# rahulrangers/P2P-Gossip-Simulation-NS3

Measured on AMD Instinct MI355X. Metric: share-deliveries/sec (edge events) at 10M nodes, 1/2/4/8 GPUs; % HBM/MFMA peak, higher is better.
Workload: dtype u64

## Files before the change

include/gossip.h:

```cpp
#ifndef GOSSIP_H
#define GOSSIP_H

#include <stdint.h>

#ifdef __cplusplus
extern "C" {
#endif

#define GOSSIP_OK 0
#define GOSSIP_EINVAL (-1)
#define GOSSIP_EHIP (-2)
#define GOSSIP_ENOMEM (-3)
#define GOSSIP_ESTATE (-4)
#define GOSSIP_ECAPACITY (-5)

const char* gossip_last_error(void);
const char* gossip_version(void);

int64_t gossip_seconds_to_ns(double seconds);
int64_t gossip_milliseconds_to_ns(double ms);

typedef struct gossip_topology gossip_topology;

#define GOSSIP_TOPO_EXACT 0
// ... 151 lines not shown
    uint64_t pull_sat_skips;
    uint32_t pull_sat;
    uint32_t pad0;
    uint64_t window_early_retires;
    uint64_t young_list_lines;
    uint64_t pull_items;
    uint64_t pull_gather_items;
    uint64_t dense_fused_launches;
    uint32_t young_grid;
    uint32_t young_skip_ticks;
    uint64_t pull_push_tiles;
    uint64_t pull_pushw_tiles;
    uint64_t pull_marks;
    uint64_t young_idle_ticks;
    uint64_t pull_fold_rows;
} gossip_counters;
int gossip_engine_get_counters(gossip_engine* e, gossip_counters* c);
int gossip_engine_get_rehearsal(gossip_engine* e, uint32_t ranges, double* pull_ms, double* pack_ms,
                                double* unpack_ms, uint64_t* msg_bytes, uint64_t* ticks);
int gossip_engine_get_rehearsal_peak(gossip_engine* e, uint32_t ranges, uint64_t* msg_bytes_max);
int gossip_engine_reset_timing(gossip_engine* e);

uint64_t gossip_engine_trace_size(const gossip_engine* e);
int gossip_engine_get_trace(const gossip_engine* e, uint32_t* node, uint32_t* share_id,
                            int64_t* tick, uint32_t* hop, uint8_t* via_recv);

void gossip_engine_destroy(gossip_engine* e);

int64_t gossip_format_event_log(const gossip_topology* t, uint64_t num_events,
                                const gossip_gen_event* ev, uint64_t num_trace,
// ... 25 lines not shown
```

p2p-gossip-simulation-ns3_amd/csrc/engine.hip:

```cpp
#include <hip/hip_runtime.h>
#include <hipcub/hipcub.hpp>
#include <rccl/rccl.h>

#include <algorithm>
#include <atomic>
#include <cstdlib>
#include <cstring>
#include <memory>
#include <mutex>
#include <new>
#include <numeric>
#include <queue>
#include <string>
#include <chrono>
#include <thread>
#include <type_traits>
#include <unordered_map>
#include <vector>

#include "internal.h"

using gossip::set_error;

namespace {
// ... 58 lines not shown
    const unsigned long long* nz_cur;
    unsigned long long* nz_next;
    uint32_t ntw;
    uint32_t v0 = 0;
    uint32_t shared_out = 0;
    uint32_t keep_lds = 0;
    uint32_t gate_seen = 1;
    const uint16_t* ptile = nullptr;
    uint32_t nptile = 0;
    unsigned long long* sat = nullptr;
    const unsigned long long* tmask = nullptr;
    const unsigned long long* mark_cur = nullptr;
    unsigned long long* mark_next = nullptr;
    uint32_t short_batch = 0;
    uint32_t fold = 0;
};

__device__ __forceinline__ uint64_t group_of(uint32_t b, uint64_t gm, uint64_t gs) {
    const uint64_t below = gs & (b == 63u ? ~0ull : ((2ull << b) - 1ull));
    const uint32_t s = 63u - (uint32_t)__builtin_clzll(below);
    const uint64_t above = gs & (s == 63u ? 0ull : ~((2ull << s) - 1ull));
    const uint64_t upto = above ? ((above & (~above + 1ull)) - 1ull) : ~0ull;
    return gm & upto & ~((1ull << s) - 1ull);
}
__device__ __forceinline__ uint64_t group_fix(uint64_t nw, uint64_t seen, uint64_t gm,
                                              uint64_t gs) {
    uint64_t todo = nw & gm;
    while (todo) {
        const uint64_t grp = group_of((uint32_t)__builtin_ctzll(todo), gm, gs);
        if (seen & grp) {
// ... 28 lines not shown
    return (uint32_t)__builtin_amdgcn_readlane((int)v, (int)src);
}
__device__ __forceinline__ uint32_t wave_sum32(uint32_t x) {
    x += (uint32_t)__builtin_amdgcn_update_dpp(0, (int)x, 0xB1, 0xF, 0xF, false);
    x += (uint32_t)__builtin_amdgcn_update_dpp(0, (int)x, 0x4E, 0xF, 0xF, false);
    x += (uint32_t)__builtin_amdgcn_update_dpp(0, (int)x, 0x141, 0xF, 0xF, false);
    x += (uint32_t)__builtin_amdgcn_update_dpp(0, (int)x, 0x140, 0xF, 0xF, false);
    return lane_read(x, 0) + lane_read(x, 16) + lane_read(x, 32) + lane_read(x, 48);
}

#include "pull_kernel.h"
#include "dense_kernel.h"
#include "young_kernel.h"

constexpr uint64_t kPullNtBytes = 16ull << 30;

int64_t env_option(const char* name, int64_t dflt) {
    const char* e = std::getenv(name);
    return e && *e ? (int64_t)std::atoll(e) : dflt;
}

uint64_t pull_grid_cap(bool nt, int64_t ov) {
    if (ov > 0) return (uint64_t)ov;
    return nt ? 16384ull : 4096ull;
}

constexpr int kWideLanes = 32;

bool pull_sp(int lpw, int epn, const PullArgs& a);
template <int LPW, bool SHORT, bool FOLD>
void launch_pull_sp(bool nt, bool push, uint32_t grid, size_t lds, hipStream_t s, const PullArgs& a) {
    if (nt && push)
        k_pull<LPW, 1, true, true, true, SHORT, FOLD><<<grid, 256, lds, s>>>(a);
    else if (nt)
        k_pull<LPW, 1, true, true, false, SHORT, FOLD><<<grid, 256, lds, s>>>(a);
    else if (push)
        k_pull<LPW, 1, false, true, true, SHORT, FOLD><<<grid, 256, lds, s>>>(a);
    else
        k_pull<LPW, 1, false, true, false, SHORT, FOLD><<<grid, 256, lds, s>>>(a);
}
template <int LPW, int EPN>
void launch_pull_t(bool nt, uint32_t grid, size_t lds, hipStream_t s, const PullArgs& a) {
    if constexpr (LPW == 32 && EPN == 1) {
        if (pull_sp(LPW, EPN, a)) {
            const bool push = a.mark_cur != nullptr || a.mark_next != nullptr;
            if (a.short_batch && a.fold)
                launch_pull_sp<LPW, true, true>(nt, push, grid, lds, s, a);
            else if (a.short_batch)
                launch_pull_sp<LPW, true, false>(nt, push, grid, lds, s, a);
            else if (a.fold)
                launch_pull_sp<LPW, false, true>(nt, push, grid, lds, s, a);
            else
                launch_pull_sp<LPW, false, false>(nt, push, grid, lds, s, a);
            return;
        }
    }
    if constexpr ((LPW == 64 || LPW == 32 || LPW == 16) && EPN == 1) {
        if (nt) {
            k_pull<LPW, 1, true><<<grid, 256, lds, s>>>(a);
            return;
// ... 481 lines not shown
    int64_t opt_seen_fold = -1;
    std::vector<int64_t> tile_lastborn;
    std::vector<int64_t> tile_foldw;
    std::vector<uint8_t> tile_folded;
    bool fold_barred = false;
    std::vector<uint8_t> fold_launch;
    std::vector<uint8_t> tr_foldw, tr_seenf;
    bool any_folded() const {
        for (size_t tl = 0; tl < tile_folded.size() && tl < tile_alloc.size(); tl++)
            if (tile_alloc[tl] && tile_folded[tl]) return true;
        return false;
    }
    int64_t opt_pull_push = -1;
    int64_t opt_peer_order = 1;
    int64_t opt_pull_batch = 0;
    std::vector<int64_t> tile_pushw;
    std::vector<std::vector<std::pair<int64_t, uint32_t>>> tile_births;
    void note_birth(uint32_t tl, int64_t t) {
        auto& h = tile_births[tl];
        if (!h.empty() && h.back().first == t)
            h.back().second++;
        else
            h.emplace_back(t, 1u);
    }
    unsigned long long* d_mark[2] = {nullptr, nullptr};
    uint64_t push_tiles = 0, pushw_tiles = 0;
    int64_t mark_tick = INT64_MIN;
    uint64_t mark_launches = 0;
    bool push_write(uint32_t tl, int64_t t) const;
    double frontier_entries(uint32_t tl, int64_t t) const;
    std::vector<int64_t> tile_inj_prev;
    std::vector<uint32_t> tile_cols;
    std::vector<double> hop_front;
    uint32_t last_lpw = 0, last_dense_tiles = 0;
    uint64_t sat_launches = 0;
    bool dense_row_hop(uint32_t tl, int64_t hop) const;
    void mark_inject(uint32_t tl, int64_t t) {
        if (tile_last_inject[tl] != t) {
            tile_inj_prev[tl] = tile_last_inject[tl];
            tile_last_inject[tl] = t;
        }
    }
    int64_t opt_young_nt = 1;
    int64_t opt_young_skip = -1;
    bool skip_wr_last = false;
    uint64_t skip_ticks = 0;
    int64_t opt_young_idle = 1;
    uint64_t idle_ticks = 0;
// ... 106 lines not shown
    int decode_trace(int64_t t);
    hipEvent_t get_event();
};

gossip_engine::~gossip_engine() {
    if (xstream) hipStreamSynchronize(xstream);
    if (stream) hipStreamSynchronize(stream);
    for (auto& p : timers) {
        hipEventDestroy(p.first);
        hipEventDestroy(p.second);
    }
    for (auto e : event_pool) hipEventDestroy(e);
    hipFree(d_rowptr); hipFree(d_col); hipFree(d_deg);
    hipFree(d_rowptr_c); hipFree(d_col_c); hipFree(d_degc);
    for (int k = 0; k < 4; k++) { hipFree(d_smask[k]); hipHostFree(h_smask[k]); }
    hipFree(d_F[0]); hipFree(d_F[1]); hipFree(d_seen_mem); hipFree(d_nz[0]); hipFree(d_nz[1]); hipFree(d_sat); hipFree(d_mark[0]); hipFree(d_mark[1]); hipFree(d_Ab); hipFree(d_FT[0]); hipFree(d_FT[1]); hipFree(d_snz[0]); hipFree(d_snz[1]); hipFree(d_snz[2]); hipFree(d_tix); hipFree(d_inc); hipFree(d_ftmsg); hipFree(d_ftrecv);
    hipFree(d_recv); hipFree(d_gen); hipFree(d_effgen); hipFree(d_sent); hipFree(d_phase_ts);
    hipFree(d_live[0]); hipFree(d_live[1]); hipFree(d_live[2]); hipFree(d_scalars); hipFree(d_acct);
    hipFree(d_msg); hipFree(d_cnt); hipFree(d_scan_tmp); hipFree(d_recv_msgs); hipFree(d_sizes);
    hipFree(d_tot); hipFree(d_ovf); hipHostFree(h_tot);
    for (int k = 0; k < kRing; k++) { hipFree(d_ptile[k]); hipHostFree(h_ptile[k]); }
    for (int k = 0; k < kRing; k++) { hipFree(d_tmask[k]); hipHostFree(h_tmask[k]); }
    hipFree(d_slot[0]); hipFree(d_slot[1]);
    hipFree(d_rev); hipFree(d_hint[0]); hipFree(d_hint[1]); hipFree(d_ylist); hipFree(d_ywork);
    for (int k = 0; k < kRing; k++) { hipFree(d_young[k]); hipHostFree(h_young[k]); }
    for (auto& p : timers_young) {
        hipEventDestroy(p.first);
        hipEventDestroy(p.second);
    }
    if (comm && !aborted.load()) ncclCommDestroy(comm);
    for (int k = 0; k < kRing; k++) {
// ... 320 lines not shown
    d_seen = d_seen_mem - (uint64_t)seen_lo * stride;
    HIP_TRY(hipMemsetAsync(d_F[0], 0, bm, stream));
    HIP_TRY(hipMemsetAsync(d_F[1], 0, bm, stream));
    HIP_TRY(hipMemsetAsync(d_seen_mem, 0, bm_seen, stream));
    {
        ntw = (stride + 1023u) / 1024u;
        const size_t nzb = (size_t)n * ntw * 8;
        for (int k = 0; k < 2; k++) {
            HIP_TRY(hipMalloc(&d_nz[k], nzb));
            HIP_TRY(hipMemsetAsync(d_nz[k], 0, nzb, stream));
        }
        if (!dense) {
            HIP_TRY(hipMalloc(&d_sat, nzb));
            HIP_TRY(hipMemsetAsync(d_sat, 0, nzb, stream));
        }
        if (!dense && row_count == 1 && !handshake)
            for (int k = 0; k < 2; k++) {
                HIP_TRY(hipMalloc(&d_mark[k], ((size_t)n + 64) / 64 * 8));
                HIP_TRY(hipMemsetAsync(d_mark[k], 0, ((size_t)n + 64) / 64 * 8, stream));
            }
    }
    {
        hop_front.clear();
        const double avg_deg = n ? (double)nnz / n : 0.0;
        double reached = n ? 1.0 / n : 0.0, front = reached;
        for (int h = 0; h < 64 && front > 0.0; h++) {
            hop_front.push_back(front);
            const double nx = (1.0 - reached) * (1.0 - std::exp(-avg_deg * front));
            reached += nx;
            front = nx;
        }
    }
    HIP_TRY(hipMalloc(&d_recv, (size_t)n * 4));
    HIP_TRY(hipMalloc(&d_gen, (size_t)n * 4));
    HIP_TRY(hipMalloc(&d_effgen, (size_t)n * 4));
    HIP_TRY(hipMalloc(&d_sent, (size_t)n * 8));
    {
        const unsigned long long init[6] = {~0ull, 0ull, 0ull, 0ull, ~0ull, 0ull};
        HIP_TRY(hipMalloc(&d_phase_ts, sizeof(init)));
        HIP_TRY(hipMemcpy(d_phase_ts, init, sizeof(init), hipMemcpyHostToDevice));
    }
    HIP_TRY(hipMemsetAsync(d_recv, 0, (size_t)n * 4, stream));
// ... 311 lines not shown
    return (double)tile_cols[tl] * hop_front[(size_t)hop] >= kDenseRowBits;
}

double gossip_engine::frontier_entries(uint32_t tl, int64_t t) const {
    double e = 0.0;
    for (const auto& b : tile_births[tl]) {
        const int64_t h = t - b.first;
        if (h >= 0 && h < (int64_t)hop_front.size()) e += (double)b.second * hop_front[(size_t)h];
    }
    return e;
}
bool gossip_engine::push_write(uint32_t tl, int64_t t) const {
    if (opt_pull_push == 1) return true;
    const double avg_deg = n ? (double)nnz / n : 0.0;
    return 1.0 - std::exp(-frontier_entries(tl, t) * avg_deg) < kPushFrac;
}

uint32_t gossip_engine::soft_cap() const {
    const uint32_t margin = std::max<uint32_t>(2u * kTileWords, stride / 16u / kTileWords * kTileWords);
    return stride > margin ? stride - margin : 0u;
}

int gossip_engine::retire_early(int64_t t) {
    if (row_count > 1 || batch) return GOSSIP_OK;
    const int64_t kt = t - 1;
    const int ls = (int)(((kt % kRing) + kRing) % kRing);
    if (kt < tick0 || !live_pending[ls] || live_tick[ls] != kt) return GOSSIP_OK;
    HIP_TRY(hipEventSynchronize(live_done[ls]));
    live_pending[ls] = false;
    early_retires++;
// ... 335 lines not shown
    const bool fold_ok = opt_seen_fold != 0 && sat_on && dr_used && !fold_barred && !handshake && !batch &&
                         !link_timing && opt_rehearse_rows <= 1;
    auto sat_window = [&](uint32_t wb) {
        const uint32_t wl = std::min(kPullLdsWords, hw - wb);
        int lpw = 8;
        while (lpw < 64 && 2 * lpw < (int)wl) lpw *= 2;
        if (lpw == 64) return true;
        const double avg_deg = n ? (double)nnz / n : 0.0;
        return !(lpw * 2 <= 64 && 8 < avg_deg);
    };
    if (trace) {
        tr_foldw.assign(hw / kTileWords, 0);
        tr_seenf.assign(hw / kTileWords, 0);
    }
    fold_launch.assign((hw + kPullLdsWords - 1) / kPullLdsWords, 0);
    if (sat_used || dr_used) {
        if (TM_WORDS * ntw > tmask_cap) {
            HIP_TRY(hipStreamSynchronize(stream));
            const uint32_t cap = TM_WORDS * std::max<uint32_t>(ntw, 8u);
            for (int k = 0; k < kRing; k++) {
                hipFree(d_tmask[k]);
                hipHostFree(h_tmask[k]);
                HIP_TRY(hipMalloc(&d_tmask[k], (size_t)cap * 8));
                HIP_TRY(hipHostMalloc(&h_tmask[k], (size_t)cap * 8, hipHostMallocDefault));
            }
            tmask_cap = cap;
        }
        unsigned long long* TM = h_tmask[slot];
        std::memset(TM, 0, (size_t)TM_WORDS * ntw * 8);
        const uint32_t ntiles = hw / kTileWords;
// ... 29 lines not shown
                m[TM_FOLDW] |= bit;
                tile_foldw[tl] = t;
                tile_folded[tl] = 1;
            }
            if (seenf || foldw) {
                fold_launch[tl * kTileWords / kPullLdsWords] = 1;
                if (trace) {
                    tr_foldw[tl] = foldw;
                    tr_seenf[tl] = seenf;
                }
            }
            if (opt_pull_batch && !fresh && tile_cols[tl] &&
                frontier_entries(tl, t - 1) >= 0.5 * (double)tile_cols[tl]) {
                m[TM_SHORT] |= bit;
                short_any = true;
            }
            if (push_on && !dr && !fresh && tile_pushw[tl] == t - 1) {
                m[TM_PUSH] |= bit;
                push_tiles++;
            }
            if (light_next && !dw && push_write(tl, t)) {
                m[TM_PUSHW] |= bit;
                pushw_any = true;
            }
            tile_listed[tl] = t;
        }
        if (dr_used && young)
            for (uint32_t i = 0; i < ny_leave; i++) {
                YoungTile& y = YP->yt[YP->lv[i]];
                if (dense_row_hop(y.tile, t - tile_first[y.tile])) {
// ... 103 lines not shown
                    c.ptile = d_ptile[slot] + pt_off[li];
                    c.nptile = pt_cnt[li];
                }
                int lpw = 8;
                while (lpw < 64 && 2 * lpw < (int)c.wact) lpw *= 2;
                const bool wide_window = lpw == 64 && split_edges;
                if (wide_window) lpw = kWideLanes;
                int epn = 1;
                while (split_edges && !wide_window && lpw * epn * 2 <= 64 && epn * 8 < avg_deg) epn *= 2;
                size_t extra_lds = 0;
                if (c.ptile && epn == 1 && (sat_used || dr_used)) {
                    c.tmask = d_tmask[slot];
                    c.sat = sat_used ? d_sat : nullptr;
                    c.short_batch = short_any ? 1u : 0u;
                    c.fold = (sat_used && li < fold_launch.size() && fold_launch[li]) ? 1u : 0u;
                    if (push_on && pull_sp(lpw, epn, c)) {
                        c.mark_cur = mark_tick == t - 1 ? d_mark[(t - 1) & 1] : nullptr;
                        mark_launches += c.mark_cur != nullptr;
                        c.mark_next = pushw_any ? d_mark[t & 1] : nullptr;
                        if (c.mark_next)
                            for (uint32_t tl = wb / kTileWords; tl < (wb + c.wact) / kTileWords; tl++)
                                if ((h_tmask[slot][(size_t)TM_WORDS * (tl >> 6) + TM_PUSHW] >> (tl & 63u)) & 1ull) {
                                    tile_pushw[tl] = t;
                                    pushw_tiles++;
                                }
                    }
                    extra_lds = kPullSatLds + ((c.mark_cur || c.mark_next) ? kPullPushLds : 0);
                    sat_launches += sat_used;
                    if (sat_used)
                        for (uint32_t tl = wb / kTileWords; tl < (wb + c.wact) / kTileWords; tl++)
// ... 923 lines not shown
        e->opt_pull_gate = env_option("GOSSIP_PULL_GATE", 1);
        e->opt_pull_tiles = env_option("GOSSIP_PULL_TILES", 1);
        e->opt_pull_tile_order = env_option("GOSSIP_PULL_TILE_ORDER", 1);
        e->opt_young_nt = env_option("GOSSIP_YOUNG_NT", 1);
        e->opt_young_skip = env_option("GOSSIP_YOUNG_SKIP", -1);
        e->opt_pull_push = env_option("GOSSIP_PULL_PUSH", -1);
        e->opt_young_idle = env_option("GOSSIP_YOUNG_IDLE", 1);
        e->opt_mem_limit = env_option("GOSSIP_MEM_LIMIT", 0);
        e->opt_xchunks = env_option("GOSSIP_XCHUNKS", 4);
        e->opt_late_age = env_option("GOSSIP_LATE_AGE", -1);
        e->opt_pull_sat = env_option("GOSSIP_PULL_SAT", 1);
        e->opt_dense_rows = env_option("GOSSIP_DENSE_ROWS", -1);
        e->opt_peer_order = env_option("GOSSIP_PEER_ORDER", 1) != 0 ? 1 : 0;
        e->opt_pull_batch = env_option("GOSSIP_PULL_BATCH", 0) != 0 ? 1 : 0;
        e->opt_seen_fold = std::max<int64_t>(-1, std::min<int64_t>(1, env_option("GOSSIP_SEEN_FOLD", -1)));
        e->trace = (cfg->flags & GOSSIP_F_TRACE) != 0;
        e->dense = cfg->mode == GOSSIP_MODE_DENSE;
        e->handshake = (cfg->flags & GOSSIP_F_HANDSHAKE) != 0;
        e->batch = (cfg->flags & GOSSIP_F_HOP_BATCH) != 0;
        if (e->batch && e->handshake)
            return set_error(GOSSIP_EINVAL, "GOSSIP_F_HOP_BATCH and GOSSIP_F_HANDSHAKE are exclusive");
        if (e->handshake) {
            if (e->dense) return set_error(GOSSIP_EINVAL, "GOSSIP_F_HANDSHAKE: CSR mode only");
            if (e->t0 < 0 || e->t0 % e->L != 0)
                return set_error(GOSSIP_EINVAL, "GOSSIP_F_HANDSHAKE: t_start must be a multiple of the latency");
            if (cfg->t_cut_ns < e->t0 + 3 * e->L)
                return set_error(GOSSIP_EINVAL, "GOSSIP_F_HANDSHAKE: t_cut must be >= t_start + 3 latency");
        }
        *out = e.release();
        return GOSSIP_OK;
// ... 362 lines not shown
        if (value < 0 || value > 1) return set_error(GOSSIP_EINVAL, "young_nt: 0 or 1");
        e->opt_young_nt = value;
    } else if (k == "young_idle") {
        if (value < 0 || value > 1) return set_error(GOSSIP_EINVAL, "young_idle: 0 or 1");
        e->opt_young_idle = value;
    } else if (k == "pull_push") {
        if (value < -1 || value > 1) return set_error(GOSSIP_EINVAL, "pull_push: -1 (auto), 0 or 1");
        e->opt_pull_push = value;
    } else if (k == "peer_order") {
        if (value < 0 || value > 1) return set_error(GOSSIP_EINVAL, "peer_order: 0 or 1");
        if (e->have_graph) return set_error(GOSSIP_ESTATE, "peer_order: set before the graph");
        e->opt_peer_order = value;
    } else if (k == "pull_batch") {
        if (value < 0 || value > 1) return set_error(GOSSIP_EINVAL, "pull_batch: 0 or 1");
        e->opt_pull_batch = value;
    } else if (k == "young_skip") {
        if (value < -1 || value > 1) return set_error(GOSSIP_EINVAL, "young_skip: -1 (auto), 0 or 1");
        e->opt_young_skip = value;
    } else if (k == "young_grid") {
        if (value < 0 || value > (1 << 20)) return set_error(GOSSIP_EINVAL, "young_grid: 0 .. 2^20 blocks");
        e->opt_young_grid = value;
    } else if (k == "mem_limit") {
        if (value < 0) return set_error(GOSSIP_EINVAL, "mem_limit >= 0 bytes");
        if (e->have_sched) return set_error(GOSSIP_ESTATE, "mem_limit: set before the schedule");
        e->opt_mem_limit = value;
    } else if (k == "late_age") {
        if (value < -1 || value > 1000) return set_error(GOSSIP_EINVAL, "late_age: -1 (auto), 0 (off) .. 1000 ticks");
        e->opt_late_age = value;
    } else if (k == "xchunks") {
        if (value < 1 || value > (int64_t)gossip_engine::kMaxChunks) return set_error(GOSSIP_EINVAL, "xchunks: 1 .. 16 row chunks");
// ... 20 lines not shown

int gossip_engine_get_option(const gossip_engine* e, const char* name, int64_t* value) {
    if (!e || !name || !value) return set_error(GOSSIP_EINVAL, "NULL argument");
    const std::string k(name);
    const std::pair<const char*, int64_t> opts[] = {
        {"pull_nt", e->opt_pull_nt}, {"pull_grid", e->opt_pull_grid},
        {"young", e->opt_young}, {"young_age", e->opt_young_age},
        {"young_cap", e->opt_young_cap}, {"young_overlap", e->opt_young_overlap},
        {"pull_tile_order", e->opt_pull_tile_order}, {"pull_tiles", e->opt_pull_tiles},
        {"pull_sat", e->opt_pull_sat}, {"dense_rows", e->opt_dense_rows}, {"pull_gate", e->opt_pull_gate},
        {"young_list_cap", e->opt_young_list_cap}, {"young_nt", e->opt_young_nt},
        {"young_skip", e->opt_young_skip}, {"pull_push", e->opt_pull_push}, {"young_idle", e->opt_young_idle}, {"young_grid", e->opt_young_grid}, {"mem_limit", e->opt_mem_limit}, {"late_age", e->opt_late_age},
        {"xchunks", e->opt_xchunks}, {"rehearse_rows", e->opt_rehearse_rows},
        {"dense_fused", e->opt_dense_fused}, {"dense_min_tiles", e->opt_dense_min_tiles},
        {"peer_order", e->opt_peer_order}, {"pull_batch", e->opt_pull_batch},
        {"seen_fold", e->opt_seen_fold}};
    for (const auto& o : opts)
        if (k == o.first) {
            *value = o.second;
            return GOSSIP_OK;
        }
    return set_error(GOSSIP_EINVAL, "unknown option '" + k + "'");
}

static int check_stepping(gossip_engine* e) {
    if (!e) return set_error(GOSSIP_EINVAL, "NULL engine");
    if (e->aborted.load()) return set_error(GOSSIP_ESTATE, "engine aborted (gossip_engine_abort)");
    if (!e->have_sched) return set_error(GOSSIP_ESTATE, "set graph and schedule first");
    if (e->comm) return set_error(GOSSIP_ESTATE, "host-staged stepping is not for an RCCL-connected engine");
    return GOSSIP_OK;
}
// ... 439 lines not shown
    c->pull_lpw = e->last_lpw;
    c->pull_dense_tiles = e->last_dense_tiles;
    c->pull_sat_skips = acct[16];
    c->pull_items = acct[20];
    c->pull_gather_items = acct[21];
    c->dense_fused_launches = e->fused_launches;
    c->young_grid = e->last_young_grid;
    c->young_skip_ticks = (uint32_t)e->skip_ticks;
    c->young_idle_ticks = e->idle_ticks;
    c->pull_push_tiles = e->push_tiles;
    c->pull_pushw_tiles = e->pushw_tiles;
    c->pull_marks = acct[32];
    c->pull_sat = e->sat_used ? 1u : 0u;
    c->window_early_retires = e->early_retires;
    c->pull_fold_rows = acct[33];
    uint64_t g = 0;
    const uint64_t done = (uint64_t)std::max<int64_t>(0, std::min(e->cur, e->tick_end) - e->tick0);
    if (!e->tick_lo.empty()) g = e->tick_lo[std::min<uint64_t>(done, e->tick_lo.size() - 1)];
    c->generations = g;
    return GOSSIP_OK;
}

int gossip_engine_get_rehearsal(gossip_engine* e, uint32_t ranges, double* pull_ms, double* pack_ms,
                                double* unpack_ms, uint64_t* msg_bytes, uint64_t* ticks) {
    if (!e) return set_error(GOSSIP_EINVAL, "NULL engine");
    if (e->opt_rehearse_rows < 2 || ranges != (uint32_t)e->opt_rehearse_rows)
        return set_error(GOSSIP_EINVAL, "get_rehearsal: ranges must equal the rehearse_rows option");
    HIP_TRY(hipSetDevice(e->device));
    HIP_TRY(hipStreamSynchronize(e->stream));
    e->rehearse_harvest();
// ... 86 lines not shown
```

p2p-gossip-simulation-ns3_amd/csrc/pull_kernel.h:

```cpp
#pragma once

__device__ __forceinline__ unsigned long long wave_sum(unsigned long long x) {
    for (int off = 32; off > 0; off >>= 1) x += __shfl_xor(x, off, 64);
    return x;
}

__device__ __forceinline__ uint32_t wave_count(bool c) { return (uint32_t)__popcll(__ballot(c)); }

template <int CTRL>
__device__ __forceinline__ uint32_t dpp_or_step(uint32_t x) {
    return x | (uint32_t)__builtin_amdgcn_update_dpp(0, (int)x, CTRL, 0xF, 0xF, false);
}
template <int G>
__device__ __forceinline__ uint32_t group_or(uint32_t x, uint32_t lane) {
    static_assert(G >= 1 && G <= 64 && (G & (G - 1)) == 0, "group size");
    if constexpr (G >= 2) x = dpp_or_step<0xB1>(x);
    if constexpr (G >= 4) x = dpp_or_step<0x4E>(x);
    if constexpr (G >= 8) x = dpp_or_step<0x141>(x);
    if constexpr (G >= 16) x = dpp_or_step<0x140>(x);
    if constexpr (G >= 32) x |= lane_get(x, lane ^ 16u);
    if constexpr (G >= 64) x |= lane_get(x, lane ^ 32u);
    return x;
}
template <int G>
// ... 3 lines not shown
}
template <int G>
__device__ __forceinline__ uint32_t group_add(uint32_t x, uint32_t lane) {
    if constexpr (G >= 2) x += (uint32_t)__builtin_amdgcn_update_dpp(0, (int)x, 0xB1, 0xF, 0xF, false);
    if constexpr (G >= 4) x += (uint32_t)__builtin_amdgcn_update_dpp(0, (int)x, 0x4E, 0xF, 0xF, false);
    if constexpr (G >= 8) x += (uint32_t)__builtin_amdgcn_update_dpp(0, (int)x, 0x141, 0xF, 0xF, false);
    if constexpr (G >= 16) x += (uint32_t)__builtin_amdgcn_update_dpp(0, (int)x, 0x140, 0xF, 0xF, false);
    if constexpr (G >= 32) x += lane_get(x, lane ^ 16u);
    if constexpr (G >= 64) x += lane_get(x, lane ^ 32u);
    return x;
}

enum : uint32_t { WF_CLEAR = 1u, WF_GROUP = 2u, WF_KEEP = 4u, WF_SNAP = 8u, WF_YOUNG = 16u, WF_LATE = 32u,
                  WF_DW = 64u, WF_BIRTH = 128u };
enum : uint32_t { TM_DENSE = 0, TM_SATOK = 1, TM_NZ = 2, TM_PUSH = 3, TM_PUSHW = 4, TM_SHORT = 5, TM_FOLDW = 6,
                  TM_SEENF = 7, TM_WORDS = 8 };
constexpr uint32_t kTmSlots = 16;

constexpr uint32_t kPullLdsWords = 2048;
#ifndef PULL_INFLIGHT
#define PULL_INFLIGHT 6
#endif
constexpr int kInflight = PULL_INFLIGHT;
#ifndef PULL_SHORT_B0
#define PULL_SHORT_B0 4
#define PULL_SHORT_B1 3
#endif
#ifndef PULL_SHORT_EVERY
#define PULL_SHORT_EVERY 0
#endif
constexpr int kShortB0 = PULL_SHORT_B0 < kInflight ? PULL_SHORT_B0 : kInflight;
constexpr int kShortB1 = PULL_SHORT_B1 < kInflight ? PULL_SHORT_B1 : kInflight;
// ... 11 lines not shown
__device__ __forceinline__ void store_row16(uint64_t* p, uint64_t x, uint64_t y) {
    if constexpr (NT) {
        unsigned long long* q = reinterpret_cast<unsigned long long*>(p);
        __builtin_nontemporal_store((unsigned long long)x, q);
        __builtin_nontemporal_store((unsigned long long)y, q + 1);
    } else {
        *reinterpret_cast<ulonglong2*>(p) = make_ulonglong2(x, y);
    }
}

__host__ __device__ constexpr size_t pull_lds_bytes(uint32_t wact, bool keep = false, uint32_t nptile = 0) {
    return (size_t)wact * 16u + (((size_t)wact + 15u) & ~(size_t)15u) + (keep ? (size_t)wact * 8u : 0u) +
           (((size_t)nptile * 2u + 15u) & ~(size_t)15u);
}
constexpr uint32_t kPullMaxPasses = 32;
constexpr size_t kPullSatLds = kTmSlots * 8u + 4u * 64u * 2u * 8u + kPullMaxPasses * 8u + 16u + 4u * kPullMaxPasses * 4u + 4u * 8u;
constexpr size_t kPullPushLds = 4u * 64u * 2u * 8u;
static_assert(2u * TM_WORDS <= kTmSlots, "tmask words of a launch fit their LDS slot");
constexpr uint32_t kNoWord = 0xffffffffu;

template <int LPW, int EPN>
__device__ __forceinline__ uint32_t pull_cid_load(const PullArgs& a, uint32_t step, uint64_t c0,
                                                  int64_t rp, int64_t rp_end, uint32_t gl,
                                                  uint32_t slot) {
    constexpr int NPW = 64 / (LPW * EPN);
    const uint32_t idx = step * NPW + slot;
    const int32_t beg = (int32_t)lane_get((uint32_t)rp, idx);
    const int32_t nx = (int32_t)lane_get((uint32_t)rp, (idx + 1u) & 63u);
    const int32_t end = (idx + 1u < 64u) ? nx : (int32_t)rp_end;
    const int32_t jj = beg + (int32_t)gl;
    return (c0 + idx < a.n && jj < end) ? (uint32_t)a.col[jj] : 0xffffffffu;
}

template <int LPW, int EPN, bool NT = false, bool SP = false, bool PUSH = false, bool SHORT = false, bool FOLD = false>
__global__ __launch_bounds__(256) __attribute__((amdgpu_waves_per_eu(SP ? 5 : 1))) void k_pull(PullArgs a) {
    static_assert(SP || !PUSH, "push marks run in the SP instantiation");
    static_assert(SP || !SHORT, "the batch schedule runs in the SP instantiation");
    static_assert(SP || !FOLD, "the SP launch picks the folding instantiation");
    constexpr bool FOLDC = FOLD || (!SP && EPN == 1);
    const bool noskip = SP ? false : a.noskip != 0u;
    constexpr int GRP = LPW * EPN;
    constexpr int NPW = 64 / GRP;
    static_assert(GRP <= 64 && (64 % GRP) == 0, "lane layout");
    extern __shared__ unsigned long long smem[];
    unsigned long long* s_lp = smem;
    unsigned long long* s_new = smem + a.wact;
    uint8_t* s_wf = reinterpret_cast<uint8_t*>(smem + 2u * a.wact);
    unsigned long long* s_keep = smem + 2u * a.wact + ((a.wact + 15u) & ~15u) / 8u;
    uint16_t* s_pt = reinterpret_cast<uint16_t*>(s_keep + (a.keep_lds ? a.wact : 0u));
    for (uint32_t i = threadIdx.x; i < a.wact; i += 256) {
        const uint8_t f = a.wflags[a.wbase + i];
        s_lp[i] = (f & WF_YOUNG) ? 0ull : (a.live_prev && !noskip) ? a.live_prev[a.wbase + i] : ~0ull;
        s_new[i] = 0ull;
        s_wf[i] = (f & WF_YOUNG) ? (uint8_t)0 : f;
        if (a.keep_lds) s_keep[i] = (f & WF_KEEP) ? a.ctl[a.wbase + i].keep : ~0ull;
    }
    for (uint32_t i = threadIdx.x; i < a.nptile; i += 256) s_pt[i] = a.ptile[i];
    const bool tm_on = SP || (EPN == 1 && a.tmask != nullptr && a.ptile != nullptr);
    const bool sat_on = SP || (tm_on && a.sat != nullptr);
    unsigned long long* s_tm = reinterpret_cast<unsigned long long*>(
        reinterpret_cast<char*>(smem) + pull_lds_bytes(a.wact, a.keep_lds != 0, a.nptile));
    unsigned long long* s_sat = s_tm + kTmSlots;
    unsigned long long* s_plm = s_sat + 4u * 128u;
    uint32_t* s_pforce = reinterpret_cast<uint32_t*>(s_plm + kPullMaxPasses);
    uint32_t* s_smask = s_pforce + 4;
    unsigned long long* s_mkw = reinterpret_cast<unsigned long long*>(s_smask + 4u * kPullMaxPasses) + wave_in_block();
    if (PUSH && (threadIdx.x & 63u) == 0u) *s_mkw = 0ull;
    unsigned long long* s_psk = s_mkw - wave_in_block() + 4u + (uint64_t)wave_in_block() * 128u;
    if (threadIdx.x < 2u * TM_WORDS) {
        const uint32_t twg = (a.wbase >> 10) + threadIdx.x / TM_WORDS;
        s_tm[threadIdx.x] = (tm_on && twg < a.ntw) ? a.tmask[twg * TM_WORDS + threadIdx.x % TM_WORDS] : 0ull;
    }
    constexpr uint32_t TPP_ = LPW >= 8 ? (uint32_t)LPW / 8u : 1u;
    const bool skip_on = SP || (tm_on && a.nptile / TPP_ <= kPullMaxPasses);
    __syncthreads();
    if (skip_on && threadIdx.x < 64u) {
        const uint32_t p = threadIdx.x, np = a.nptile / TPP_;
        unsigned long long lm = 0ull;
        bool force = false, last = p + 1u == np;
        bool sh_any = false, sh_all = true;
        if (p < np) {
            for (uint32_t k = 0; k < TPP_; k++) {
                const uint32_t t = s_pt[p * TPP_ + k];
                if (t == 0xffffu) continue;
                if constexpr (SHORT) {
                    const uint32_t tg = (a.wbase >> 4) + t;
                    const uint32_t q = (tg >> 6) - (a.wbase >> 10);
                    const bool sh = q < 2u && ((s_tm[q * TM_WORDS + TM_SHORT] >> (tg & 63u)) & 1ull) != 0ull;
                    sh_any |= sh;
                    sh_all &= sh;
                }
                unsigned long long lv = 0ull;
                uint32_t fl = 0u;
                for (uint32_t q = 0; q < 16u; q++) {
                    lv |= s_lp[t * 16u + q];
                    fl |= s_wf[t * 16u + q];
                }
                if (lv) lm |= 1ull << (((a.wbase >> 4) + t) & 63u);
                if (fl & (WF_CLEAR | WF_DW | WF_KEEP)) force = true;
            }
            if (p + 1u < np && ((a.wbase + (uint32_t)s_pt[(p + 1u) * TPP_] * 16u) >> 10) !=
                                   ((a.wbase + (uint32_t)s_pt[p * TPP_] * 16u) >> 10))
                last = true;
            s_plm[p] = lm;
        }
        const unsigned long long fm = __ballot(p < np && force), lmk = __ballot(p < np && last);
        const unsigned long long tq = __ballot(p < np && ((a.wbase + (uint32_t)s_pt[p * TPP_] * 16u) >> 10) != (a.wbase >> 10));
        const unsigned long long t0 = __ballot(p < np && ((a.wbase + (uint32_t)s_pt[p * TPP_] * 16u) >> 10) == (a.wbase >> 10));
        const unsigned long long shm = __ballot(p < np && (PULL_SHORT_EVERY ? sh_any && sh_all : sh_any));
        if (threadIdx.x == 0) {
            if constexpr (SHORT) s_pforce[3] = (uint32_t)shm;
            s_pforce[0] = (uint32_t)fm;
            s_pforce[1] = (uint32_t)lmk;
            s_pforce[2] = (t0 ? 1u : 0u) | (tq ? 2u : 0u);
        }
    }
    __syncthreads();
    const uint32_t lane_id = threadIdx.x & 63u;
#define PULL_LANES                                                                             \
    const uint32_t lane = opaque(lane_id);                                                    \
    const uint32_t gl = lane % GRP, wl = gl % LPW, el = gl / LPW, slot = lane / GRP;          \
    (void)el;
    const uint64_t stride = a.stride;
    const uint64_t n = a.n;
    const uint64_t wave = (uint64_t)blockIdx.x * 4u + wave_in_block();
// ... 16 lines not shown
        if (!listed) return (uint32_t)(nzw >> (((a.wbase + p * 2u * LPW) >> 4) & 63u)) & 0xffu;
        uint32_t r = 0;
#pragma unroll
        for (uint32_t k = 0; k < TPP; k++) {
            const uint32_t t = s_pt[p * TPP + k];
            if (t != 0xffffu) r |= (uint32_t)((nzw >> (((a.wbase >> 4) + t) & 63u)) & 1ull) << k;
        }
        return r;
    };
    const uint32_t nsteps = 64u / NPW;
    unsigned long long snap_local = 0ull;
    uint32_t t_pe = 0, t_col = 0, t_srd = 0, t_swr = 0, t_fwr = 0, t_nz = 0, t_sk = 0;
    uint32_t t_it = 0, t_gi = 0;
    uint32_t t_mk = 0;
    uint32_t t_fold = 0;
    unsigned long long nzacc = 0ull;
    const bool gather = EPN == 1;
    const uint32_t tw_base = a.wbase >> 10;
    unsigned long long* s_satw = s_sat + (uint64_t)wave_in_block() * 128u;
    auto satv_of = [&](uint32_t idx, uint32_t tw) -> unsigned long long {
        return sat_on ? s_satw[idx * 2u + (tw - tw_base)] : 0ull;
    };
    auto nz_needed = [&](uint32_t idx, uint32_t tw) -> bool {
        return !tm_on || (s_tm[(tw - tw_base) * TM_WORDS + TM_NZ] & ~satv_of(idx, tw)) != 0ull;
    };

    auto tm_bit = [&](uint32_t which, uint32_t tw, uint32_t wg) -> bool {
        if constexpr (!FOLDC) return false;
        return sat_on && ((s_tm[(tw - tw_base) * TM_WORDS + which] >> ((wg >> 4) & 63u)) & 1ull) != 0ull;
    };
// ... 172 lines not shown
            if (act && (f1 & WF_KEEP)) k1 = s_keep[w + 1 - a.wbase];
            const uint64_t want0 = lp0 & ~s2.x & k0, want1 = lp1 & ~s2.y & k1;
            const bool need = act && !dead && !s2c_gated && (noskip || (want0 | want1) != 0ull);
            int tn = need ? 1 : 0;
            tn = (int)group_or<8>((uint32_t)tn, lane);
            const bool tneed = tn != 0 && act;
            int gneed = tn;
            gneed = (int)group_or<GRP>((uint32_t)gneed, lane);
            t_it += wave_count(gl == 0 && c0 + idx < n);
            t_gi += wave_count(gl == 0 && gneed != 0);
            uint64_t acc0 = 0ull, acc1 = 0ull;
            if (gneed) {
                const uint64_t* Fw = a.Fcur + w;
                if constexpr (EPN == 1) {
                    const bool late = ((f0 | f1) & WF_LATE) != 0u;
                    auto gchunk = [&](uint32_t cid, unsigned long long nzw, int rem, uint32_t sh) {
                        t_col += wave_count((int)gl < rem);
                        const uint32_t nzp = pass_bits(nzw | drm, pass);
                        int bs = kInflight;
                        for (int t0 = 0; t0 < rem; t0 += bs) {
                            if constexpr (SHORT)
                                bs = !sh ? kInflight : t0 == 0 ? kShortB0 : t0 == kShortB0 ? kShortB1 : kInflight;
                            const int lim = SHORT ? min(rem, t0 + bs) : rem;
                            int open = (noskip || !late)
                                           ? 1 : (((want0 & ~acc0) | (want1 & ~acc1)) != 0ull);
                            open = (int)group_or<8>((uint32_t)open, lane);
                            int gopen = open;
                            gopen = (int)group_or<GRP>((uint32_t)gopen, lane);
                            if (!gopen) break;
                            uint32_t u[kInflight], z[kInflight];
#pragma unroll
                            for (int t = 0; t < kInflight; t++) {
                                const uint32_t src = (lane & ~(uint32_t)(GRP - 1)) | ((uint32_t)(t0 + t) & (GRP - 1u));
// ... 4 lines not shown
#pragma unroll
                            for (int t = 0; t < kInflight; t++) {
                                q[t] = make_ulonglong2(0ull, 0ull);
                                const bool issue = open && tneed && t0 + t < lim && ((z[t] >> (wl >> 3)) & 1u);
                                if (issue) q[t] = load_row16<NT>(Fw + (uint64_t)u[t] * stride);
                                t_pe += wave_count(issue);
                            }
#pragma unroll
                            for (int t = 0; t < kInflight; t++) {
                                acc0 |= q[t].x;
                                acc1 |= q[t].y;
                            }
                        }
                    };
                    const uint32_t shortp = SHORT ? (uint32_t)__builtin_amdgcn_readfirstlane((int)((s_pforce[3] >> pass) & 1u)) : 0u;
                    gchunk(cid0, nz0, min(GRP, end - beg), shortp);
                    for (int32_t cb = beg + GRP; cb < end; cb += GRP) {
                        const int rem = min(GRP, end - cb);
                        const int32_t jj = cb + (int32_t)gl;
                        const uint32_t cid = (jj < end) ? (uint32_t)a.col[jj] : 0u;
                        const bool ld = (int)gl < rem && nz_needed(idx, tw);
                        const unsigned long long nzw = ld ? a.nz_cur[(uint64_t)cid * a.ntw + tw] : 0ull;
                        t_nz += wave_count(ld);
                        gchunk(cid, nzw, rem, 0u);
                    }
                } else {
                    for (int32_t j0 = beg + (int32_t)el; j0 < end; j0 += 8 * EPN) {
                        uint32_t u[8];
                        unsigned long long z[8];
#pragma unroll
                        for (int t = 0; t < 8; t++) {
                            const int32_t j = j0 + t * EPN;
                            u[t] = (tneed && j < end) ? (uint32_t)a.col[j] : 0xffffffffu;
                            t_col += wave_count(wl == 0 && u[t] != 0xffffffffu);
                        }
#pragma unroll
                        for (int t = 0; t < 8; t++) {
                            z[t] = 0ull;
                            if (u[t] != 0xffffffffu) z[t] = a.nz_cur[(uint64_t)u[t] * a.ntw + tw];
// ... 125 lines not shown
                const int32_t e = j + 1u < 64u ? (int32_t)lane_read((uint32_t)rp, j + 1u) : (int32_t)rp_end;
                for (int32_t q = b + (int32_t)lane_id; q < e; q += 64) {
                    const uint32_t u = (uint32_t)a.col[q];
                    atomicOr(&a.mark_next[u >> 6], 1ull << (u & 63u));
                    nm++;
                }
            }
            t_mk += wave_sum32(nm);
        }
    }
    if (a.snap) {
        snap_local = wave_sum(snap_local);
        if (lane_id == 0 && snap_local) atomicAdd(a.snap, snap_local);
    }
    if (a.acct && lane_id == 0) {
        const uint32_t tv[11] = {t_pe, t_col, t_srd, t_swr, t_fwr, t_nz, t_sk, t_it, t_gi, t_mk, t_fold};
        const int slot_of[11] = {0, 1, 2, 3, 4, 7, 16, 20, 21, 32, 33};
#pragma unroll
        for (int q = 0; q < 11; q++)
            if (tv[q]) acct_add(a.acct, (uint32_t)slot_of[q], (unsigned long long)tv[q]);
    }
    __syncthreads();
    for (uint32_t i = threadIdx.x; i < a.wact; i += 256) {
        const unsigned long long x = s_new[i];
        if (x) atomicOr(&a.live[a.wbase + i], x);
    }
#undef PULL_LANES
}

#ifdef PULL_DIAG_SKIP_ENV
#include <cstdlib>
static inline bool diag_skip_tile(int64_t age) {
    static const long a = std::getenv("GOSSIP_DIAG_SKIP_AGE") ? std::atol(std::getenv("GOSSIP_DIAG_SKIP_AGE")) : 0;
    return a > 0 && age >= a;
// ... 6 lines not shown
```

p2p-gossip-simulation-ns3_amd/gossip/__init__.py:

```python
from __future__ import annotations

import ctypes as C
import os
from dataclasses import dataclass

import numpy as np

_HERE = os.path.dirname(os.path.abspath(__file__))
LIB_DIR = os.path.join(os.path.dirname(_HERE), "lib")
LIB_PATH = os.environ.get("GOSSIP_LIB_PATH") or os.path.join(LIB_DIR, "libgossip.so")

TOPO_EXACT = 0
TOPO_SKIP = 1
MODE_AUTO = 0
MODE_CSR = 1
MODE_DENSE = 2
F_TRACE = 1
F_TIMING = 2
F_NOSKIP = 4
F_TILE_PER_TICK = 32
F_HANDSHAKE = 64
F_HOP_BATCH = 128
F_SHARD_BY_TICK = 256

# ... 62 lines not shown
        ("young_col_ids", C.c_uint64), ("young_fallback_rows", C.c_uint64),
        ("young_seen_reads", C.c_uint64), ("young_seen_writes", C.c_uint64),
        ("young_rows_written", C.c_uint64), ("young_slot_writes", C.c_uint64),
        ("exchange_bytes_sent", C.c_uint64), ("exchange_bytes_received", C.c_uint64),
        ("pull_phase_ms", C.c_double), ("young_line2_misses", C.c_uint64),
        ("pull_late_age", C.c_uint32), ("pull_tiles", C.c_uint32),
        ("young_fresh_lines", C.c_uint64),
        ("pull_lpw", C.c_uint32), ("pull_dense_tiles", C.c_uint32),
        ("pull_sat_skips", C.c_uint64), ("pull_sat", C.c_uint32), ("pad0", C.c_uint32),
        ("window_early_retires", C.c_uint64), ("young_list_lines", C.c_uint64),
        ("pull_items", C.c_uint64), ("pull_gather_items", C.c_uint64),
        ("dense_fused_launches", C.c_uint64),
        ("young_grid", C.c_uint32), ("young_skip_ticks", C.c_uint32),
        ("pull_push_tiles", C.c_uint64), ("pull_pushw_tiles", C.c_uint64), ("pull_marks", C.c_uint64),
        ("young_idle_ticks", C.c_uint64), ("pull_fold_rows", C.c_uint64),
    ]


_lib = None


def _ptr(a, ct):
    return a.ctypes.data_as(C.POINTER(ct)) if a is not None else None


def load_library(path: str = LIB_PATH):
    global _lib
    if _lib is not None:
        return _lib
    if not os.path.exists(path):
# ... 591 lines not shown
```

Before: 18880 billion.

## Add rolling software-pipelined gather for pull tiles predicted to need all neighbor rows

Adds a ROLL instantiation of the sparse pull kernel. For chunks whose tiles are flagged, it keeps kInflight row loads in flight and refills each slot as it is consumed, instead of loading in batches with early-exit checks. Lanes with nothing to load read a shared zero row, so loads can be issued without branching. A host-side model built from hop frontier and seen fractions chooses which tiles use the rolling path by default. The cost is extra loads, since early termination is lost, plus more LDS and tmask slots and more template instantiations.

Measured after the change: 18820 billion. No clear change (-0.3%).

```diff
diff --git a/include/gossip.h b/include/gossip.h
--- a/include/gossip.h
+++ b/include/gossip.h
@@ -189,6 +189,8 @@
     uint64_t pull_marks;
     uint64_t young_idle_ticks;
     uint64_t pull_fold_rows;
+    uint64_t pull_roll_items;
+    uint64_t pull_roll_rows;
 } gossip_counters;
 int gossip_engine_get_counters(gossip_engine* e, gossip_counters* c);
 int gossip_engine_get_rehearsal(gossip_engine* e, uint32_t ranges, double* pull_ms, double* pack_ms,
diff --git a/p2p-gossip-simulation-ns3_amd/csrc/engine.hip b/p2p-gossip-simulation-ns3_amd/csrc/engine.hip
--- a/p2p-gossip-simulation-ns3_amd/csrc/engine.hip
+++ b/p2p-gossip-simulation-ns3_amd/csrc/engine.hip
@@ -96,6 +96,8 @@
     unsigned long long* mark_next = nullptr;
     uint32_t short_batch = 0;
     uint32_t fold = 0;
+    uint32_t roll = 0;
+    const uint64_t* zrow = nullptr;
 };
 
 __device__ __forceinline__ uint64_t group_of(uint32_t b, uint64_t gm, uint64_t gs) {
@@ -154,6 +156,9 @@
 #include "young_kernel.h"
 
 constexpr uint64_t kPullNtBytes = 16ull << 30;
+
+constexpr int64_t kPullRollDefault = -1;
+inline int64_t pull_roll_value(int64_t v) { return (v == -1 || v == 0 || v == 2) ? v : kPullRollDefault; }
 
 int64_t env_option(const char* name, int64_t dflt) {
     const char* e = std::getenv(name);
@@ -184,6 +189,17 @@
     if constexpr (LPW == 32 && EPN == 1) {
         if (pull_sp(LPW, EPN, a)) {
             const bool push = a.mark_cur != nullptr || a.mark_next != nullptr;
+            if (a.roll && a.zrow && !push && !a.short_batch) {
+                if (nt && a.fold)
+                    k_pull<LPW, 1, true, true, false, false, true, true><<<grid, 256, lds, s>>>(a);
+                else if (nt)
+                    k_pull<LPW, 1, true, true, false, false, false, true><<<grid, 256, lds, s>>>(a);
+                else if (a.fold)
+                    k_pull<LPW, 1, false, true, false, false, true, true><<<grid, 256, lds, s>>>(a);
+                else
+                    k_pull<LPW, 1, false, true, false, false, false, true><<<grid, 256, lds, s>>>(a);
+                return;
+            }
             if (a.short_batch && a.fold)
                 launch_pull_sp<LPW, true, true>(nt, push, grid, lds, s, a);
             else if (a.short_batch)
@@ -695,6 +711,10 @@
     int64_t opt_pull_push = -1;
     int64_t opt_peer_order = 1;
     int64_t opt_pull_batch = 0;
+    int64_t opt_pull_roll = kPullRollDefault;
+    bool roll_tile(uint32_t tl, int64_t t) const;
+    std::vector<uint8_t> roll_launch;
+    uint64_t* d_zrow = nullptr;
     std::vector<int64_t> tile_pushw;
     std::vector<std::vector<std::pair<int64_t, uint32_t>>> tile_births;
     void note_birth(uint32_t tl, int64_t t) {
@@ -713,6 +733,7 @@
     std::vector<int64_t> tile_inj_prev;
     std::vector<uint32_t> tile_cols;
     std::vector<double> hop_front;
+    std::vector<double> hop_seen;
     uint32_t last_lpw = 0, last_dense_tiles = 0;
     uint64_t sat_launches = 0;
     bool dense_row_hop(uint32_t tl, int64_t hop) const;
@@ -849,7 +870,7 @@
     hipFree(d_rowptr); hipFree(d_col); hipFree(d_deg);
     hipFree(d_rowptr_c); hipFree(d_col_c); hipFree(d_degc);
     for (int k = 0; k < 4; k++) { hipFree(d_smask[k]); hipHostFree(h_smask[k]); }
-    hipFree(d_F[0]); hipFree(d_F[1]); hipFree(d_seen_mem); hipFree(d_nz[0]); hipFree(d_nz[1]); hipFree(d_sat); hipFree(d_mark[0]); hipFree(d_mark[1]); hipFree(d_Ab); hipFree(d_FT[0]); hipFree(d_FT[1]); hipFree(d_snz[0]); hipFree(d_snz[1]); hipFree(d_snz[2]); hipFree(d_tix); hipFree(d_inc); hipFree(d_ftmsg); hipFree(d_ftrecv);
+    hipFree(d_F[0]); hipFree(d_F[1]); hipFree(d_seen_mem); hipFree(d_nz[0]); hipFree(d_nz[1]); hipFree(d_sat); hipFree(d_zrow); hipFree(d_mark[0]); hipFree(d_mark[1]); hipFree(d_Ab); hipFree(d_FT[0]); hipFree(d_FT[1]); hipFree(d_snz[0]); hipFree(d_snz[1]); hipFree(d_snz[2]); hipFree(d_tix); hipFree(d_inc); hipFree(d_ftmsg); hipFree(d_ftrecv);
     hipFree(d_recv); hipFree(d_gen); hipFree(d_effgen); hipFree(d_sent); hipFree(d_phase_ts);
     hipFree(d_live[0]); hipFree(d_live[1]); hipFree(d_live[2]); hipFree(d_scalars); hipFree(d_acct);
     hipFree(d_msg); hipFree(d_cnt); hipFree(d_scan_tmp); hipFree(d_recv_msgs); hipFree(d_sizes);
@@ -1200,6 +1221,10 @@
             HIP_TRY(hipMalloc(&d_sat, nzb));
             HIP_TRY(hipMemsetAsync(d_sat, 0, nzb, stream));
         }
+        if (!dense) {
+            HIP_TRY(hipMalloc(&d_zrow, 128));
+            HIP_TRY(hipMemsetAsync(d_zrow, 0, 128, stream));
+        }
         if (!dense && row_count == 1 && !handshake)
             for (int k = 0; k < 2; k++) {
                 HIP_TRY(hipMalloc(&d_mark[k], ((size_t)n + 64) / 64 * 8));
@@ -1208,10 +1233,12 @@
     }
     {
         hop_front.clear();
+        hop_seen.clear();
         const double avg_deg = n ? (double)nnz / n : 0.0;
         double reached = n ? 1.0 / n : 0.0, front = reached;
         for (int h = 0; h < 64 && front > 0.0; h++) {
             hop_front.push_back(front);
+            hop_seen.push_back(reached);
             const double nx = (1.0 - reached) * (1.0 - std::exp(-avg_deg * front));
             reached += nx;
             front = nx;
@@ -1553,6 +1580,19 @@
     if (opt_pull_push == 1) return true;
     const double avg_deg = n ? (double)nnz / n : 0.0;
     return 1.0 - std::exp(-frontier_entries(tl, t) * avg_deg) < kPushFrac;
+}
+
+constexpr double kRollCols = 8.0;
+bool gossip_engine::roll_tile(uint32_t tl, int64_t t) const {
+    const double avg_deg = n ? (double)nnz / n : 0.0;
+    const double rows = std::max(0.0, avg_deg + 2.0 * std::sqrt(avg_deg) - (double)kInflight);
+    double e = 0.0;
+    for (const auto& b : tile_births[tl]) {
+        const int64_t h = t - 1 - b.first;
+        if (h < 0 || h >= (int64_t)hop_front.size()) continue;
+        e += (double)b.second * (1.0 - hop_seen[(size_t)h]) * std::pow(1.0 - hop_front[(size_t)h], rows);
+    }
+    return e >= kRollCols;
 }
 
 uint32_t gossip_engine::soft_cap() const {
@@ -1918,6 +1958,7 @@
         tr_seenf.assign(hw / kTileWords, 0);
     }
     fold_launch.assign((hw + kPullLdsWords - 1) / kPullLdsWords, 0);
+    roll_launch.assign((hw + kPullLdsWords - 1) / kPullLdsWords, 0);
     if (sat_used || dr_used) {
         if (TM_WORDS * ntw > tmask_cap) {
             HIP_TRY(hipStreamSynchronize(stream));
@@ -1977,6 +2018,10 @@
                 frontier_entries(tl, t - 1) >= 0.5 * (double)tile_cols[tl]) {
                 m[TM_SHORT] |= bit;
                 short_any = true;
+            }
+            if (sat_used && d_zrow && (opt_pull_roll == 2 || (opt_pull_roll == -1 && dr && roll_tile(tl, t)))) {
+                m[TM_ROLL] |= bit;
+                roll_launch[tl * kTileWords / kPullLdsWords] = 1;
             }
             if (push_on && !dr && !fresh && tile_pushw[tl] == t - 1) {
                 m[TM_PUSH] |= bit;
@@ -2110,6 +2155,8 @@
                     c.sat = sat_used ? d_sat : nullptr;
                     c.short_batch = short_any ? 1u : 0u;
                     c.fold = (sat_used && li < fold_launch.size() && fold_launch[li]) ? 1u : 0u;
+                    c.roll = (sat_used && li < roll_launch.size() && roll_launch[li]) ? 1u : 0u;
+                    c.zrow = d_zrow;
                     if (push_on && pull_sp(lpw, epn, c)) {
                         c.mark_cur = mark_tick == t - 1 ? d_mark[(t - 1) & 1] : nullptr;
                         mark_launches += c.mark_cur != nullptr;
@@ -3063,6 +3110,7 @@
         e->opt_peer_order = env_option("GOSSIP_PEER_ORDER", 1) != 0 ? 1 : 0;
         e->opt_pull_batch = env_option("GOSSIP_PULL_BATCH", 0) != 0 ? 1 : 0;
         e->opt_seen_fold = std::max<int64_t>(-1, std::min<int64_t>(1, env_option("GOSSIP_SEEN_FOLD", -1)));
+        e->opt_pull_roll = pull_roll_value(env_option("GOSSIP_PULL_ROLL", kPullRollDefault));
         e->trace = (cfg->flags & GOSSIP_F_TRACE) != 0;
         e->dense = cfg->mode == GOSSIP_MODE_DENSE;
         e->handshake = (cfg->flags & GOSSIP_F_HANDSHAKE) != 0;
@@ -3455,6 +3503,10 @@
     } else if (k == "pull_batch") {
         if (value < 0 || value > 1) return set_error(GOSSIP_EINVAL, "pull_batch: 0 or 1");
         e->opt_pull_batch = value;
+    } else if (k == "pull_roll") {
+        if (value != -1 && value != 0 && value != 2)
+            return set_error(GOSSIP_EINVAL, "pull_roll: -1 (auto), 0 or 2 (every gathering pass)");
+        e->opt_pull_roll = value;
     } else if (k == "young_skip") {
         if (value < -1 || value > 1) return set_error(GOSSIP_EINVAL, "young_skip: -1 (auto), 0 or 1");
         e->opt_young_skip = value;
@@ -3505,7 +3557,7 @@
         {"xchunks", e->opt_xchunks}, {"rehearse_rows", e->opt_rehearse_rows},
         {"dense_fused", e->opt_dense_fused}, {"dense_min_tiles", e->opt_dense_min_tiles},
         {"peer_order", e->opt_peer_order}, {"pull_batch", e->opt_pull_batch},
-        {"seen_fold", e->opt_seen_fold}};
+        {"seen_fold", e->opt_seen_fold}, {"pull_roll", e->opt_pull_roll}};
     for (const auto& o : opts)
         if (k == o.first) {
             *value = o.second;
@@ -3975,6 +4027,8 @@
     c->pull_sat = e->sat_used ? 1u : 0u;
     c->window_early_retires = e->early_retires;
     c->pull_fold_rows = acct[33];
+    c->pull_roll_items = acct[34];
+    c->pull_roll_rows = acct[35];
     uint64_t g = 0;
     const uint64_t done = (uint64_t)std::max<int64_t>(0, std::min(e->cur, e->tick_end) - e->tick0);
     if (!e->tick_lo.empty()) g = e->tick_lo[std::min<uint64_t>(done, e->tick_lo.size() - 1)];
diff --git a/p2p-gossip-simulation-ns3_amd/csrc/pull_kernel.h b/p2p-gossip-simulation-ns3_amd/csrc/pull_kernel.h
--- a/p2p-gossip-simulation-ns3_amd/csrc/pull_kernel.h
+++ b/p2p-gossip-simulation-ns3_amd/csrc/pull_kernel.h
@@ -41,8 +41,8 @@
 enum : uint32_t { WF_CLEAR = 1u, WF_GROUP = 2u, WF_KEEP = 4u, WF_SNAP = 8u, WF_YOUNG = 16u, WF_LATE = 32u,
                   WF_DW = 64u, WF_BIRTH = 128u };
 enum : uint32_t { TM_DENSE = 0, TM_SATOK = 1, TM_NZ = 2, TM_PUSH = 3, TM_PUSHW = 4, TM_SHORT = 5, TM_FOLDW = 6,
-                  TM_SEENF = 7, TM_WORDS = 8 };
-constexpr uint32_t kTmSlots = 16;
+                  TM_SEENF = 7, TM_ROLL = 8, TM_WORDS = 9 };
+constexpr uint32_t kTmSlots = 24;
 
 constexpr uint32_t kPullLdsWords = 2048;
 #ifndef PULL_INFLIGHT
@@ -84,7 +84,8 @@
            (((size_t)nptile * 2u + 15u) & ~(size_t)15u);
 }
 constexpr uint32_t kPullMaxPasses = 32;
-constexpr size_t kPullSatLds = kTmSlots * 8u + 4u * 64u * 2u * 8u + kPullMaxPasses * 8u + 16u + 4u * kPullMaxPasses * 4u + 4u * 8u;
+constexpr uint32_t kPforceWords = 8;
+constexpr size_t kPullSatLds = kTmSlots * 8u + 4u * 64u * 2u * 8u + kPullMaxPasses * 8u + kPforceWords * 4u + 4u * kPullMaxPasses * 4u + 4u * 8u;
 constexpr size_t kPullPushLds = 4u * 64u * 2u * 8u;
 static_assert(2u * TM_WORDS <= kTmSlots, "tmask words of a launch fit their LDS slot");
 constexpr uint32_t kNoWord = 0xffffffffu;
@@ -102,11 +103,13 @@
     return (c0 + idx < a.n && jj < end) ? (uint32_t)a.col[jj] : 0xffffffffu;
 }
 
-template <int LPW, int EPN, bool NT = false, bool SP = false, bool PUSH = false, bool SHORT = false, bool FOLD = false>
+template <int LPW, int EPN, bool NT = false, bool SP = false, bool PUSH = false, bool SHORT = false, bool FOLD = false,
+          bool ROLL = false>
 __global__ __launch_bounds__(256) __attribute__((amdgpu_waves_per_eu(SP ? 5 : 1))) void k_pull(PullArgs a) {
     static_assert(SP || !PUSH, "push marks run in the SP instantiation");
     static_assert(SP || !SHORT, "the batch schedule runs in the SP instantiation");
     static_assert(SP || !FOLD, "the SP launch picks the folding instantiation");
+    static_assert(!ROLL || (SP && !PUSH && !SHORT), "the rolling gather runs in SP instantiations of its own");
     constexpr bool FOLDC = FOLD || (!SP && EPN == 1);
     const bool noskip = SP ? false : a.noskip != 0u;
     constexpr int GRP = LPW * EPN;
@@ -133,7 +136,7 @@
     unsigned long long* s_sat = s_tm + kTmSlots;
     unsigned long long* s_plm = s_sat + 4u * 128u;
     uint32_t* s_pforce = reinterpret_cast<uint32_t*>(s_plm + kPullMaxPasses);
-    uint32_t* s_smask = s_pforce + 4;
+    uint32_t* s_smask = s_pforce + kPforceWords;
     unsigned long long* s_mkw = reinterpret_cast<unsigned long long*>(s_smask + 4u * kPullMaxPasses) + wave_in_block();
     if (PUSH && (threadIdx.x & 63u) == 0u) *s_mkw = 0ull;
     unsigned long long* s_psk = s_mkw - wave_in_block() + 4u + (uint64_t)wave_in_block() * 128u;
@@ -149,6 +152,7 @@
         unsigned long long lm = 0ull;
         bool force = false, last = p + 1u == np;
         bool sh_any = false, sh_all = true;
+        bool rl_all = true;
         if (p < np) {
             for (uint32_t k = 0; k < TPP_; k++) {
                 const uint32_t t = s_pt[p * TPP_ + k];
@@ -167,6 +171,10 @@
                     fl |= s_wf[t * 16u + q];
                 }
                 if (lv) lm |= 1ull << (((a.wbase >> 4) + t) & 63u);
+                if constexpr (ROLL) {
+                    const uint32_t tg = (a.wbase >> 4) + t, q = (tg >> 6) - (a.wbase >> 10);
+                    if (lv) rl_all &= q < 2u && ((s_tm[q * TM_WORDS + TM_ROLL] >> (tg & 63u)) & 1ull) != 0ull;
+                }
                 if (fl & (WF_CLEAR | WF_DW | WF_KEEP)) force = true;
             }
             if (p + 1u < np && ((a.wbase + (uint32_t)s_pt[(p + 1u) * TPP_] * 16u) >> 10) !=
@@ -178,7 +186,9 @@
         const unsigned long long tq = __ballot(p < np && ((a.wbase + (uint32_t)s_pt[p * TPP_] * 16u) >> 10) != (a.wbase >> 10));
         const unsigned long long t0 = __ballot(p < np && ((a.wbase + (uint32_t)s_pt[p * TPP_] * 16u) >> 10) == (a.wbase >> 10));
         const unsigned long long shm = __ballot(p < np && (PULL_SHORT_EVERY ? sh_any && sh_all : sh_any));
+        const unsigned long long rlm = ROLL ? __ballot(p < np && lm != 0ull && rl_all) : 0ull;
         if (threadIdx.x == 0) {
+            if constexpr (ROLL) s_pforce[4] = (uint32_t)rlm;
             if constexpr (SHORT) s_pforce[3] = (uint32_t)shm;
             s_pforce[0] = (uint32_t)fm;
             s_pforce[1] = (uint32_t)lmk;
@@ -225,6 +235,7 @@
     uint32_t t_it = 0, t_gi = 0;
     uint32_t t_mk = 0;
     uint32_t t_fold = 0;
+    uint32_t t_ri = 0, t_rp = 0;
     unsigned long long nzacc = 0ull;
     const bool gather = EPN == 1;
     const uint32_t tw_base = a.wbase >> 10;
@@ -427,9 +438,39 @@
                 const uint64_t* Fw = a.Fcur + w;
                 if constexpr (EPN == 1) {
                     const bool late = ((f0 | f1) & WF_LATE) != 0u;
-                    auto gchunk = [&](uint32_t cid, unsigned long long nzw, int rem, uint32_t sh) {
+                    auto gchunk = [&](uint32_t cid, unsigned long long nzw, int rem, uint32_t sh, bool rl) {
                         t_col += wave_count((int)gl < rem);
                         const uint32_t nzp = pass_bits(nzw | drm, pass);
+                        if constexpr (ROLL) {
+                            if (rl) {
+                                const uint32_t pe0 = t_pe;
+                                auto rload = [&](int t) -> ulonglong2 {
+                                    const uint32_t src = (lane & ~(uint32_t)(GRP - 1)) | ((uint32_t)t & (GRP - 1u));
+                                    const uint32_t u = lane_get(cid, src), z = lane_get(nzp, src);
+                                    const bool issue = tneed && t < rem && ((z >> (wl >> 3)) & 1u);
+                                    t_pe += wave_count(issue);
+                                    return load_row16<NT>(issue ? Fw + (uint64_t)u * stride : a.zrow);
+                                };
+                                ulonglong2 q[kInflight];
+#pragma unroll
+                                for (int t = 0; t < kInflight; t++) q[t] = rload(t);
+#pragma unroll
+                                for (int t = kInflight; t < GRP; t++) {
+                                    if (__ballot(t < rem) == 0ull) break;
+                                    acc0 |= q[t % kInflight].x;
+                                    acc1 |= q[t % kInflight].y;
+                                    q[t % kInflight] = rload(t);
+                                }
+#pragma unroll
+                                for (int t = 0; t < kInflight; t++) {
+                                    acc0 |= q[t].x;
+                                    acc1 |= q[t].y;
+                                }
+                                t_ri += wave_count(gl == 0);
+                                t_rp += t_pe - pe0;
+                                return;
+                            }
+                        }
                         int bs = kInflight;
                         for (int t0 = 0; t0 < rem; t0 += bs) {
                             if constexpr (SHORT)
@@ -464,7 +505,8 @@
                         }
                     };
                     const uint32_t shortp = SHORT ? (uint32_t)__builtin_amdgcn_readfirstlane((int)((s_pforce[3] >> pass) & 1u)) : 0u;
-                    gchunk(cid0, nz0, min(GRP, end - beg), shortp);
+                    const bool rollp = ROLL && __builtin_amdgcn_readfirstlane((int)((s_pforce[4] >> pass) & 1u)) != 0;
+                    gchunk(cid0, nz0, min(GRP, end - beg), shortp, rollp);
                     for (int32_t cb = beg + GRP; cb < end; cb += GRP) {
                         const int rem = min(GRP, end - cb);
                         const int32_t jj = cb + (int32_t)gl;
@@ -472,7 +514,7 @@
                         const bool ld = (int)gl < rem && nz_needed(idx, tw);
                         const unsigned long long nzw = ld ? a.nz_cur[(uint64_t)cid * a.ntw + tw] : 0ull;
                         t_nz += wave_count(ld);
-                        gchunk(cid, nzw, rem, 0u);
+                        gchunk(cid, nzw, rem, 0u, false);
                     }
                 } else {
                     for (int32_t j0 = beg + (int32_t)el; j0 < end; j0 += 8 * EPN) {
@@ -628,10 +670,10 @@
         if (lane_id == 0 && snap_local) atomicAdd(a.snap, snap_local);
     }
     if (a.acct && lane_id == 0) {
-        const uint32_t tv[11] = {t_pe, t_col, t_srd, t_swr, t_fwr, t_nz, t_sk, t_it, t_gi, t_mk, t_fold};
-        const int slot_of[11] = {0, 1, 2, 3, 4, 7, 16, 20, 21, 32, 33};
-#pragma unroll
-        for (int q = 0; q < 11; q++)
+        const uint32_t tv[13] = {t_pe, t_col, t_srd, t_swr, t_fwr, t_nz, t_sk, t_it, t_gi, t_mk, t_fold, t_ri, t_rp};
+        const int slot_of[13] = {0, 1, 2, 3, 4, 7, 16, 20, 21, 32, 33, 34, 35};
+#pragma unroll
+        for (int q = 0; q < 13; q++)
             if (tv[q]) acct_add(a.acct, (uint32_t)slot_of[q], (unsigned long long)tv[q]);
     }
     __syncthreads();
diff --git a/p2p-gossip-simulation-ns3_amd/gossip/__init__.py b/p2p-gossip-simulation-ns3_amd/gossip/__init__.py
--- a/p2p-gossip-simulation-ns3_amd/gossip/__init__.py
+++ b/p2p-gossip-simulation-ns3_amd/gossip/__init__.py
@@ -100,6 +100,7 @@
         ("young_grid", C.c_uint32), ("young_skip_ticks", C.c_uint32),
         ("pull_push_tiles", C.c_uint64), ("pull_pushw_tiles", C.c_uint64), ("pull_marks", C.c_uint64),
         ("young_idle_ticks", C.c_uint64), ("pull_fold_rows", C.c_uint64),
+        ("pull_roll_items", C.c_uint64), ("pull_roll_rows", C.c_uint64),
     ]
 
 
```
